# Dorothy-2016/rgbd360

Hardware: AMD Instinct MI355X
Metric: registered Frame360 pairs/sec @ 8×640×480; ICP-reduce HBM GB/s vs roofline (higher is better)
Workload: dtype f32

## Files before the change

### include/rgbd360_hip.h

```cpp
#ifndef RGBD360_HIP_H
#define RGBD360_HIP_H
#include <stddef.h>
#include <stdint.h>

#ifdef __cplusplus
extern "C" {
#endif

#define R360_NUM_SENSORS 8
#define R360_MAX_PYR 6

typedef struct r360_ctx r360_ctx;
typedef struct r360_calib r360_calib;
typedef struct r360_frame r360_frame;

int         r360_ctx_create(int device, r360_ctx** out);
void        r360_ctx_destroy(r360_ctx* ctx);
int         r360_ctx_sync(r360_ctx* ctx);
void*       r360_ctx_stream(r360_ctx* ctx);
const char* r360_last_error(void);
const char* r360_version(void);
const char* r360_data_dir(void);

int  r360_calib_create(r360_ctx* ctx, int rows, int cols, r360_calib** out);
// ... 253 lines not shown
    float pbmap_info[36];
    int   dense_rc;
    float pose[16];
    float hessian[36];
    r360_icp_stats stats;
} r360_pair_result;

int r360_batch_register(r360_batch* b, const r360_pair_job* jobs, int n, size_t max_match_planes, int mode,
                        int min_matches, float min_area, const r360_icp_params* p, r360_pair_result* out);

int r360_track_frame(r360_batch* b, r360_frame* const* kfs, int n_kf, r360_frame* frame, int num_check,
                     int no_assoc_threshold, size_t max_match_planes, int mode, int* chosen,
                     r360_pair_result* result, r360_pair_result* cand);

typedef struct {
    int   label, count, start_idx, n_contour, n_fit;
    float centroid[3], cov[9], model[4], curvature;
} r360_region;
int r360_frame_get_cloud(r360_frame* f, float* xyz4, uint8_t* rgb4, float* nrm4, float* dist);
int r360_frame_get_labels(r360_frame* f, int* lab, int* labf);
int r360_frame_get_regions(r360_frame* f, int sensor, r360_region* out, int cap, int* n);
int r360_frame_segment_eval(r360_frame* f, const float* xyz4, const float* nrm, int nrm_comps, const uint8_t* rgb4,
                            int* err_code);
int r360_frame_get_region_detail(r360_frame* f, int sensor, int region, int64_t* stats, float* bounds,
                                 float* contour4, int cap, int* n_contour);

typedef struct r360_comm r360_comm;
int  r360_comm_unique_id(uint8_t id[128]);
int  r360_comm_init(int device, int nranks, int rank, const uint8_t id[128], r360_comm** out);
void r360_comm_destroy(r360_comm* c);
int  r360_comm_allgather(r360_comm* c, const void* send, void* recv, size_t bytes);
int  r360_comm_allreduce_max(r360_comm* c, double* v, int n);

int  r360_dev_alloc(int device, size_t bytes, void** out);
int  r360_dev_free(void* p);
int  r360_dev_copy(void* dst, const void* src, size_t bytes, int kind);

int r360_synth_frame(const r360_calib* calib, uint32_t seed, const float rig_pose[16],
                     uint8_t* bgr8, uint16_t* depth8);
int r360_synth_frame_rt(int rows, int cols, const float* rt8, uint32_t seed, const float rig_pose[16],
                        uint8_t* bgr8, uint16_t* depth8);
int r360_synth_path_pose(uint32_t seed, int frame, float pose_out[16]);

int r360_proj_check(const float* X, const float* Y, const float* Z, int n, int nRows, int nCols,
                    unsigned long long* mismatches, unsigned long long* fallbacks);
int r360_proj_check_pose(const float* lx, const float* ly, const float* lz, int n, const float pose[16], int nRows,
// ... 201 lines not shown
```

### rgbd360_amd/__init__.py

```python
from __future__ import annotations

import ctypes as C
import os
import numpy as np

C = C

__all__ = [
    "lib", "Context", "Calib360", "Frame360", "RegisterPhotoICP", "RegisterRGBD360", "IcpParams", "IcpStats",
    "GicpParams", "GicpStats", "GeneralizedICP", "GraphParams", "GraphStats", "PoseGraph", "g2o_write", "g2o_read",
    "PHOTO_CONSISTENCY", "DEPTH_CONSISTENCY", "PHOTO_DEPTH", "synth_path_pose", "exp_se3",
    "LIB_PATH", "ABI_SYMBOLS", "Batch", "PairJob", "PairResult", "JOB_PBMAP_ONLY", "JOB_GATED", "JOB_ALWAYS",
    "TopoParams", "TopologicalMap", "Relocalizer", "topo_bisect", "topo_partition", "topo_partition_batch",
]

_HERE = os.path.dirname(os.path.abspath(__file__))
LIB_PATH = os.environ.get("R360_LIB") or os.path.join(_HERE, "lib", "librgbd360_hip.so")
REPO_ROOT = os.path.dirname(_HERE)

PHOTO_CONSISTENCY, DEPTH_CONSISTENCY, PHOTO_DEPTH = 0, 1, 2
BUILD_UNDISTORT, BUILD_SPHERE, BUILD_PYRAMID, BUILD_CLOUD, BUILD_PLANES = 1, 2, 4, 8, 16
BUILD_SENSOR_PYRAMID = 32
BUILD_LOCAL_PLANES = 64
BUILT_LEVEL0 = 256
# ... 303 lines not shown
    ("r360_match_params_load_ini", C.c_int, [C.c_char_p, C.POINTER(MatchParams)]),
    ("r360_ctx_set_match_params", C.c_int, [_P, C.POINTER(MatchParams)]),
    ("r360_ctx_get_match_params", C.c_int, [_P, C.POINTER(MatchParams)]),
    ("r360_ctx_match_stats", C.c_int, [_P, C.POINTER(C.c_long), C.POINTER(C.c_long), C.POINTER(C.c_long)]),
    ("r360_match_tree_search", C.c_int, [C.c_int, C.c_int, _P, _P, C.c_int, _P, C.c_long, _P, C.POINTER(C.c_long)]),
    ("r360_batch_set_match_params", C.c_int, [_P, C.POINTER(MatchParams)]),
    ("r360_register_pbmap", C.c_int, [_P, _P, _P, C.c_size_t, C.c_int, _FP, _FP, _IP, C.c_int, _IP, _FP, _FP, _FP]),
    ("r360_register", C.c_int, [_P, _P, _P, _FP, C.POINTER(IcpParams), C.c_size_t, C.c_int, _FP, _FP,
                                C.POINTER(IcpStats)]),
    ("r360_register_async", C.c_int, [_P, _P, _P, _FP, C.POINTER(IcpParams), C.c_size_t, C.c_int]),
    ("r360_register_result", C.c_int, [_P, _FP, _FP, C.POINTER(IcpStats)]),
    ("r360_pbmap_match_tables", C.c_int, [_P, _P, _P, C.c_size_t, C.c_int, _IP, _IP, _IP, _IP, _P, _P, C.c_int]),
    ("r360_batch_create", C.c_int, [C.c_int, C.c_int, C.POINTER(C.c_void_p)]),
    ("r360_batch_destroy", None, [_P]),
    ("r360_batch_lanes", C.c_int, [_P]),
    ("r360_batch_register", C.c_int, [_P, C.POINTER(PairJob), C.c_int, C.c_size_t, C.c_int, C.c_int, C.c_float,
                                      C.POINTER(IcpParams), C.POINTER(PairResult)]),
    ("r360_track_frame", C.c_int, [_P, C.POINTER(C.c_void_p), C.c_int, _P, C.c_int, C.c_int, C.c_size_t, C.c_int,
                                   _IP, C.POINTER(PairResult), C.POINTER(PairResult)]),
    ("r360_frame_get_cloud", C.c_int, [_P, _FP, _P, _FP, _FP]),
    ("r360_frame_get_labels", C.c_int, [_P, _IP, _IP]),
    ("r360_frame_get_regions", C.c_int, [_P, C.c_int, C.POINTER(Region), C.c_int, _IP]),
    ("r360_frame_segment_eval", C.c_int, [_P, _FP, _FP, C.c_int, _P, _IP]),
    ("r360_frame_get_region_detail", C.c_int, [_P, C.c_int, C.c_int, C.POINTER(C.c_int64), _FP, _FP, C.c_int, _IP]),
    ("r360_comm_unique_id", C.c_int, [_P]),
    ("r360_comm_init", C.c_int, [C.c_int, C.c_int, C.c_int, _P, C.POINTER(_P)]),
    ("r360_comm_destroy", None, [_P]),
    ("r360_comm_allgather", C.c_int, [_P, _P, _P, C.c_size_t]),
    ("r360_comm_allreduce_max", C.c_int, [_P, _DP, C.c_int]),
    ("r360_dev_alloc", C.c_int, [C.c_int, C.c_size_t, C.POINTER(_P)]),
    ("r360_dev_free", C.c_int, [_P]),
    ("r360_dev_copy", C.c_int, [_P, _P, C.c_size_t, C.c_int]),
    ("r360_synth_frame", C.c_int, [_P, C.c_uint32, _FP, _P, _P]),
    ("r360_synth_frame_rt", C.c_int, [C.c_int, C.c_int, _FP, C.c_uint32, _FP, _P, _P]),
    ("r360_synth_path_pose", C.c_int, [C.c_uint32, C.c_int, _FP]),
    ("r360_libm_eval", C.c_int, [_FP, _FP, _FP, C.c_int, _FP, _FP, C.c_int]),
    ("r360_rn_check", C.c_int, [C.c_uint, C.c_uint, C.POINTER(C.c_ulonglong)]),
    ("r360_rank6", C.c_int, [_FP, C.c_int, _IP]),
    ("r360_data_dir", C.c_char_p, []),
    ("r360_solve6", C.c_int, [_DP, _DP, C.c_int, _DP]),
    ("r360_proj_check_pose", C.c_int, [_FP, _FP, _FP, C.c_int, _FP, C.c_int, C.c_int, C.POINTER(C.c_ulonglong),
                                       C.POINTER(C.c_ulonglong)]),
    ("r360_proj_check", C.c_int, [_FP, _FP, _FP, C.c_int, C.c_int, C.c_int, C.POINTER(C.c_ulonglong),
                                  C.POINTER(C.c_ulonglong)]),
    ("r360_ctx_debug_stamps", C.c_int, [_P, C.POINTER(C.c_ulonglong)]),
    ("r360_ctx_kernel_time", C.c_int, [_P, C.c_int, C.POINTER(C.c_double), C.POINTER(C.c_long)]),
# ... 536 lines not shown
        n = C.c_int()
        arr = (Region * 64)()
        _check(lib().r360_frame_get_regions(self.h, sensor, arr, 64, C.byref(n)), "get_regions")
        return [dict(label=r.label, count=r.count, start_idx=r.start_idx, n_contour=r.n_contour, n_fit=r.n_fit,
                     centroid=np.array(r.centroid[:]), cov=np.array(r.cov[:]).reshape(3, 3),
                     model=np.array(r.model[:]), curvature=r.curvature) for r in arr[:n.value]]

    def segment_eval(self, xyz4: np.ndarray, nrm: np.ndarray, rgb4: np.ndarray) -> int:
        h, w = self.rows // 2, self.cols // 2
        xyz4 = np.ascontiguousarray(xyz4, np.float32)
        nrm = np.ascontiguousarray(nrm, np.float32)
        rgb4 = np.ascontiguousarray(rgb4, np.uint8)
        if xyz4.shape != (8, h, w, 4) or nrm.shape[:3] != (8, h, w) or nrm.shape[3] not in (3, 4) or \
                rgb4.shape != (8, h, w, 4):
            raise ValueError(f"segment_eval: fields of 8 x {h} x {w} expected")
        code = C.c_int(0)
        rc = lib().r360_frame_segment_eval(self.h, _fptr(xyz4), _fptr(nrm), nrm.shape[3], _vptr(rgb4), C.byref(code))
        if rc < 0:
            e = RuntimeError(f"segment_eval failed ({rc}): {lib().r360_last_error().decode()}")
            e.code = code.value
            raise e
        return rc

    def region_detail(self, sensor: int, region: int) -> dict:
        st = (C.c_int64 * 20)()
        bounds = np.zeros(6, np.float32)
        n = C.c_int()
        _check(lib().r360_frame_get_region_detail(self.h, sensor, region, st, _fptr(bounds), None, 0, C.byref(n)),
               "get_region_detail")
        contour = np.zeros((max(n.value, 1), 4), np.float32)
        if n.value:
            _check(lib().r360_frame_get_region_detail(self.h, sensor, region, None, None, _fptr(contour), n.value,
                                                      C.byref(n)), "get_region_detail")
        s2 = []
        for k in range(6):
            v = (int(st[4 + 2 * k]) & 0xFFFFFFFFFFFFFFFF) | ((int(st[5 + 2 * k]) & 0xFFFFFFFFFFFFFFFF) << 64)
            s2.append(v - (1 << 128) if v >> 127 else v)
        return dict(n=int(st[0]), s1=[int(st[1 + k]) for k in range(3)], s2=s2, c=[int(st[16 + k]) for k in range(4)],
                    bmin=bounds[:3].copy(), bmax=bounds[3:].copy(), contour=contour[:n.value].copy())

    def sphere(self):
        bgr = np.zeros((self.sph_rows, self.sph_cols, 3), np.uint8)
        dep = np.zeros((self.sph_rows, self.sph_cols), np.uint16)
        _check(lib().r360_frame_get_sphere(self.h, _vptr(bgr), _vptr(dep)), "get_sphere")
        return bgr, dep

# ... 131 lines not shown

    def match_tables(self, mode: int = PLANAR_3DoF, cap: int = 128):
        ns, nt = C.c_int(), C.c_int()
        sid, tid = np.zeros(cap, np.int32), np.zeros(cap, np.int32)
        un = np.zeros(cap * cap, np.uint8)
        words = (cap * cap + 63) // 64
        bi = np.zeros(cap * cap * words, np.uint64)
        _check(lib().r360_ctx_set_match_params(self.ctx.h, C.byref(self.match)), "set_match_params")
        w = _check(lib().r360_pbmap_match_tables(self.ctx.h, self.ref.h, self.trg.h, self.max_match_planes, mode,
                                                 C.byref(ns), C.byref(nt), sid.ctypes.data_as(_IP),
                                                 tid.ctypes.data_as(_IP), _vptr(un), _vptr(bi), cap), "match_tables")
        n, m = ns.value, nt.value
        return dict(sid=sid[:n].copy(), tid=tid[:m].copy(), unary=un[:n * m].reshape(n, m).copy(),
                    binary=bi[:n * m * w].reshape(n * m, w).copy(), words=w)


def frames_build(frames, flags: int = None):
    if flags is None:
        flags = BUILD_UNDISTORT | BUILD_CLOUD | BUILD_PLANES | BUILD_SPHERE | BUILD_PYRAMID
    arr = (C.c_void_p * len(frames))(*[f.h for f in frames])
    _check(lib().r360_frames_build(arr, len(frames), flags), "r360_frames_build")


def register(ctx: "Context", ref: "Frame360", trg: "Frame360", guess=None, params: "IcpParams | None" = None,
             max_match_planes: int = 25, mode: int = PLANAR_3DoF):
    g = _mat16(np.eye(4) if guess is None else guess)
    pose, info = np.zeros(16, np.float32), np.zeros(36, np.float32)
    st = IcpStats()
    p = params if params is not None else IcpParams.default()
    rc = _check(lib().r360_register(ctx.h, ref.h, trg.h, _fptr(g), C.byref(p), max_match_planes, mode, _fptr(pose),
                                    _fptr(info), C.byref(st)), "register")
    return _from16(pose), info.reshape(6, 6).T.copy(), st, rc == 0


class Batch:

    def __init__(self, device: int = 0, lanes: int = 8):
        h = C.c_void_p()
        _check(lib().r360_batch_create(device, lanes, C.byref(h)), "r360_batch_create")
        self.h = h
        self.lanes = lib().r360_batch_lanes(h)

    def register_pairs(self, jobs, max_match_planes: int = 25, mode: int = PLANAR_3DoF, min_matches: int = 0,
                       min_area: float = 0.0, params: "IcpParams | None" = None) -> list[dict]:
        jobs = list(jobs)
        arr = (PairJob * max(1, len(jobs)))()
# ... 901 lines not shown
```

### rgbd360_amd/csrc/host/pbmap.cpp

```cpp
#include <hip/hip_runtime.h>

#include <algorithm>
#include <chrono>
#include <condition_variable>
#include <deque>
#include <mutex>
#include <string>
#include <thread>
#include <cmath>
#include <cstdio>
#include <cstdlib>
#include <cstring>
#include <map>
#include <zlib.h>
#include <set>
#include <vector>

#include "../r360_internal.h"


int launch_match_tables(r360_ctx* ctx, hipStream_t stream, const float* d_desc, int ns, int nt, int mode,
                        uint8_t* d_unary, unsigned long long* d_bin, int words);

namespace {
// ... 1560 lines not shown
extern "C" int r360_frame_get_regions(r360_frame* f, int sensor, r360_region* out, int cap, int* n) {
    if (int rc = ready(f)) return rc;
    CHECK_ARG(f->pl.cloud, "frame planes were loaded, not built: no per-sensor regions");
    CHECK_ARG(sensor >= 0 && sensor < 8, "sensor out of range");
    PlaneBufs& P = f->pl;
    const int nm = P.h_nmodels[sensor];
    if (n) *n = nm;
    for (int m = 0; m < nm && m < cap && out; ++m) {
        const PlaneOut& O = P.h_out[sensor * R360_MAX_MODELS + m];
        r360_region& r = out[m];
        r.label = O.model.label;
        r.count = (int)O.stats.n;
        r.start_idx = O.start;
        r.n_contour = O.n_contour;
        r.n_fit = O.model.n_fit;
        for (int k = 0; k < 3; ++k) r.centroid[k] = O.model.centroid[k];
        for (int k = 0; k < 9; ++k) r.cov[k] = O.model.cov[k];
        for (int k = 0; k < 4; ++k) r.model[k] = O.model.v[k];
        r.curvature = O.model.curvature;
    }
    return 0;
}

extern "C" int r360_frame_segment_eval(r360_frame* f, const float* xyz4, const float* nrm, int nrm_comps,
                                       const uint8_t* rgb4, int* err_code) {
    CHECK_ARG(f && xyz4 && nrm && rgb4 && (nrm_comps == 3 || nrm_comps == 4), "segment_eval: bad arguments");
    if (bind_device(f->ctx->device)) return -1;
    CHECK_ARG(f->rows > 0, "a sphere-only frame has no sensor images");
    planes_join(f);
    if (plane_bufs_alloc(f)) return -1;
    r360_ctx* ctx = f->ctx;
    hipStream_t st = ctx->stream;
    PlaneBufs& P = f->pl;
    const int w = P.w, h = P.h, rows = f->rows, cols = f->cols;
    const size_t T = 8 * (size_t)w * h;
    std::vector<uint8_t> bgr((size_t)8 * rows * cols * 3, 0);
    for (int s = 0; s < 8; ++s)
        for (int r = 0; r < h; ++r)
            for (int c = 0; c < w; ++c) {
                const uint8_t* q = rgb4 + 4 * (((size_t)s * h + r) * w + c);
                uint8_t* d = bgr.data() + (((size_t)s * rows + 2 * r + 1) * cols + 2 * c + 1) * 3;
                d[0] = q[2]; d[1] = q[1]; d[2] = q[0];
            }
    std::vector<float> n4;
    if (nrm_comps == 3) {
        n4.resize(4 * T);
        for (size_t i = 0; i < T; ++i) {
            for (int k = 0; k < 3; ++k) n4[4 * i + k] = nrm[3 * i + k];
            n4[4 * i + 3] = 0.f;
        }
    }
    if (hipEvent_t e = f->bgr_wait()) R360_HIP(hipEventSynchronize(e));
    R360_HIP(hipStreamSynchronize(st));
    f->bgr_split = false;
    R360_HIP(hipMemcpy(f->d_bgr, bgr.data(), bgr.size(), hipMemcpyHostToDevice));
    R360_HIP(hipMemcpy(P.cloud, xyz4, sizeof(float4) * T, hipMemcpyHostToDevice));
    R360_HIP(hipMemcpy(P.nrm, nrm_comps == 3 ? n4.data() : nrm, sizeof(float4) * T, hipMemcpyHostToDevice));
    const PlaneGeom G = plane_geom(f);
    long cells, entries, groups;
    vox_scratch_need(G, &cells, &entries, &groups);
    if (ctx_vhash_reserve(ctx, cells, entries, groups)) return -1;
    PlaneBatch B;
    std::memset(&B, 0, sizeof B);
    B.f[0] = plane_dev(f, VoxScratch{ctx->d_vhash, (unsigned long long)ctx->vhash_cap, ctx->d_vlist, ctx->d_vcnt});
    P.ticket.reset();
    delete f->pbmap;
    f->pbmap = nullptr;
    delete f->local;
    f->local = nullptr;
    f->built = 0;
    if (launch_segment_inputs(B, 1, G, st)) return -1;
    if (launch_segmentation(B, 1, G, st, ctx, nullptr)) return -1;
    if (launch_plane_publish(B, 1, st)) return -1;
    R360_HIP(hipEventRecord(P.done, st));
    R360_HIP(hipStreamSynchronize(st));
    f->built = R360_BUILD_CLOUD | R360_BUILD_PLANES;
    if (err_code) *err_code = P.h_nmodels[8];
    if (planes_capacity_ok(f)) {
        P.worker_rc = -1;
        P.worker_err = r360_last_error();
        return -1;
    }
    P.worker_rc = 0;
    P.worker_err.clear();
    f->pbmap = new PbMapHost;
    return 0;
}

extern "C" int r360_frame_get_region_detail(r360_frame* f, int sensor, int region, int64_t* stats, float* bounds,
                                            float* contour4, int cap, int* n_contour) {
    if (int rc = ready(f)) return rc;
    CHECK_ARG(f->pl.cloud, "frame planes were loaded, not built: no per-sensor regions");
    CHECK_ARG(sensor >= 0 && sensor < 8, "sensor out of range");
    PlaneBufs& P = f->pl;
    CHECK_ARG(region >= 0 && region < P.h_nmodels[sensor], "region out of range");
    const PlaneOut& O = P.h_out[sensor * R360_MAX_MODELS + region];
    if (stats) {
        stats[0] = O.stats.n;
        for (int k = 0; k < 3; ++k) stats[1 + k] = O.stats.s1[k];
        for (int k = 0; k < 6; ++k) {
            const unsigned __int128 u = (unsigned __int128)O.stats.s2[k];
            stats[4 + 2 * k] = (int64_t)(unsigned long long)u;
            stats[5 + 2 * k] = (int64_t)(unsigned long long)(u >> 64);
        }
        for (int k = 0; k < 4; ++k) stats[16 + k] = O.stats.c[k];
    }
    if (bounds)
        for (int k = 0; k < 3; ++k) { bounds[k] = O.bmin[k]; bounds[3 + k] = O.bmax[k]; }
// ... 135 lines not shown
```

### rgbd360_amd/csrc/kernels/plane_seg.hip

```cpp
#include <cstdio>
#include <cstdlib>
#include <cstring>
#include <type_traits>
#include "../r360_internal.h"
#include "../plane_math.h"

namespace {

__device__ __forceinline__ bool isfin(float v) { return __builtin_isfinite(v); }

__device__ __forceinline__ int ld(const int* p) { return __hip_atomic_load(p, __ATOMIC_RELAXED, __HIP_MEMORY_SCOPE_AGENT); }

__device__ int find_root(int* parent, int x) {
    int p = ld(parent + x);
    while (p != x) {
        const int gp = ld(parent + p);
        if (gp != p) __hip_atomic_store(parent + x, gp, __ATOMIC_RELAXED, __HIP_MEMORY_SCOPE_AGENT);
        x = gp;
        p = ld(parent + x);
    }
    return x;
}

__device__ void unite(int* parent, int a, int b) {
// ... 906 lines not shown
    int8_t* B = bnd + (long)s * R360_REFINE_BANDS * w;
    int* Fl = flag + s * R360_REFINE_BANDS;
    for (int i = 1; i < nb; ++i) {
        const int b = DIR > 0 ? i : nb - 1 - i;
        const int prev = b - DIR;
        __builtin_amdgcn_fence(__ATOMIC_RELEASE, "workgroup");
        __builtin_amdgcn_wave_barrier();
        __builtin_amdgcn_fence(__ATOMIC_ACQUIRE, "workgroup");
        if (!__builtin_amdgcn_readfirstlane(Fl[prev])) continue;
        const int r0 = b * rb, r1 = min(h, r0 + rb);
        refine_band<K, DIR>(Sin + s * N, Sout + s * N, MK + s * N, w, h, r0, r1, B + (long)prev * w, B + (long)b * w,
                            Fl + b, true);
    }
}
template <int K, int DIR>
__global__ void __launch_bounds__(64) k_refine_p2(const PlaneBatch B, int w, int h, int rb, int nb) {
    const PlaneDev& D = B.f[blockIdx.z];
    d_refine_p2<K, DIR>(DIR > 0 ? D.state : D.state2, DIR > 0 ? D.state2 : D.state, D.mask, w, h, rb, nb, D.rbnd, D.rflag);
}


constexpr int RW_PF = 8;

__device__ __forceinline__ void d_refine_skew(const int8_t* __restrict__ S, const unsigned long long* __restrict__ MK, int w, int h,
                              uint16_t* __restrict__ code, unsigned long long* __restrict__ msk, int* __restrict__ fb) {
    const long N = (long)w * h, SK = (long)(h + w - 1) * h, total = 8 * SK;
    if (blockIdx.x == 0 && threadIdx.x < 24) fb[threadIdx.x] = 0;
    for (long d = blockIdx.x * (long)blockDim.x + threadIdx.x; d < total; d += (long)gridDim.x * blockDim.x) {
        const int s = (int)(d / SK);
        const long q = d - (long)s * SK;
        const int k = (int)(q / h), r = (int)(q - (long)k * h);
        const int c = k - r;
        if (c < 0 || c >= w) continue;
        const int j = r * w + c;
        const long i = (long)s * N + j;
        const int8_t* O = S + (long)s * N;
        const bool c1 = r >= 1 && c <= w - 2 && O[(r - 1) * w + c + 1] != -1;
        const bool c2 = r <= h - 2 && (c >= 1 ? O[(r + 1) * w + c - 1] != -1 : O[r * w + w - 1] != -1);
        code[d] = (uint16_t)((uint8_t)O[j] | (c1 ? 0x100 : 0) | (c2 ? 0x200 : 0));
        msk[d] = MK[i];
    }
}
__global__ void k_refine_skew(const PlaneBatch B, int w, int h) {
    const PlaneDev& D = B.f[blockIdx.z];
    d_refine_skew(D.state, D.mask, w, h, D.rcode, D.rmsk, D.rflag);
}


__device__ __forceinline__ bool mbit(unsigned long long m, int v) { return (v >= 0) & (((m >> (v & 63)) & 1ull) != 0); }

constexpr int RW_MAX_REDO = 64;

template <int DIR>
__device__ __forceinline__ void d_refine_wave(const uint16_t* __restrict__ code_all,
                                                      const unsigned long long* __restrict__ msk_all,
                                                      int8_t* __restrict__ f1_all, int8_t* __restrict__ f2_all,
                                                      int* __restrict__ fb, int w, int h) {
    __shared__ int xch[2][16];
    __shared__ int8_t wasm[1024], wdet[1024];
    __shared__ int s_red, s_min;
    __shared__ int chg[2][16];
    const int s = blockIdx.x;
    const int r = threadIdx.x, lane = r & 63, wv = r >> 6, nw = blockDim.x >> 6;
    const long SK = (long)(h + w - 1) * h;
    const uint16_t* code = code_all + s * SK;
    const unsigned long long* msk = msk_all + s * SK;
    int8_t* f1 = f1_all + s * SK;
    int8_t* f2 = f2_all + s * SK;
// ... 416 lines not shown
template <int DIR, int NW>
__global__ void __launch_bounds__(64 * NW) k_refine_pipe(const PlaneBatch B, int w, int h, int narrow_max) {
    const PlaneDev& D = B.f[blockIdx.z];
    d_refine_pipe<DIR, NW>(D.rcode, D.rmsk, D.rf1, D.rf2, D.nmodels, D.rflag, w, h, narrow_max);
}


__device__ __forceinline__ void d_refine_unskew(const int8_t* __restrict__ f2_all, int8_t* __restrict__ S_all,
                                const int* __restrict__ fb, int w, int h) {
    const long N = (long)w * h, SK = (long)(h + w - 1) * h, total = 8 * N;
    for (long i = blockIdx.x * (long)blockDim.x + threadIdx.x; i < total; i += (long)gridDim.x * blockDim.x) {
        const int s = (int)(i / N);
        if (fb[s]) continue;
        const int j = (int)(i - (long)s * N), r = j / w, c = j - r * w;
        S_all[i] = f2_all[s * SK + (long)(r + c) * h + r];
    }
}
__global__ void k_refine_unskew(const PlaneBatch B, int w, int h) {
    const PlaneDev& D = B.f[blockIdx.z];
    d_refine_unskew(D.rf2, D.state, D.rflag, w, h);
}


template <int K>
__device__ __forceinline__ void d_refine_fb(const int8_t* __restrict__ f1_all, const int8_t* __restrict__ f2_all,
                                                 int8_t* __restrict__ S_all,
                                                 const unsigned long long* __restrict__ MK, const int* __restrict__ fb,
                                                 int w, int h) {
    const int s = blockIdx.x;
    if (fb[16 + s]) {
        refine_sweeps<K>(S_all, MK, w, h, s, 3);
        return;
    }
    const int r0 = fb[s] - 1;
    if (r0 < 0) return;
    const long N = (long)w * h, SK = (long)(h + w - 1) * h;
    for (long j = threadIdx.x; j < N; j += 64) {
        const int r = (int)(j / w), c = (int)(j - (long)r * w);
        S_all[s * N + j] = (r <= r0 ? f1_all : f2_all)[s * SK + (long)(r + c) * h + r];
    }
    __builtin_amdgcn_fence(__ATOMIC_RELEASE, "workgroup");
    __builtin_amdgcn_wave_barrier();
    __builtin_amdgcn_fence(__ATOMIC_ACQUIRE, "workgroup");
    refine_sweeps<K>(S_all, MK, w, h, s, 2, r0 + 1);
}
template <int K>
__global__ void __launch_bounds__(64) k_refine_fb(const PlaneBatch B, int w, int h) {
    const PlaneDev& D = B.f[blockIdx.z];
    d_refine_fb<K>(D.rf1, D.rf2, D.state, D.mask, D.rflag, w, h);
}


__device__ __forceinline__ void d_refine_final(const int8_t* __restrict__ state, const int* __restrict__ lab, int N,
                               const PlaneModel* __restrict__ models, int* __restrict__ labf) {
    const long total = 8L * N;
    for (long i = blockIdx.x * (long)blockDim.x + threadIdx.x; i < total; i += (long)gridDim.x * blockDim.x) {
        const int s = (int)(i / N);
        const int st = state[i];
        labf[i] = st >= 0 ? models[s * R360_MAX_MODELS + st].label : (st == -2 ? lab[i] : -1);
    }
}
__global__ void k_refine_final(const PlaneBatch B, int N) {
    const PlaneDev& D = B.f[blockIdx.z];
    d_refine_final(D.state, D.lab, N, D.models, D.labf);
}


__device__ __forceinline__ void d_nbmask(const int* __restrict__ labf, int w, int h, uint8_t* __restrict__ nb,
                         const RegionPart* __restrict__ gpart, const int* __restrict__ nmodels,
                         PlaneOut* __restrict__ out) {
    const int N = w * h;
    const long total = 8L * N;
// ... 544 lines not shown
        if (keep) dst[off + (int)__builtin_amdgcn_mbcnt_hi((unsigned)(bal >> 32), __builtin_amdgcn_mbcnt_lo((unsigned)bal, 0u))] = v;
        __syncthreads();
        if (tid == 0) for (int w = 0; w < VOXH_TPB / 64; ++w) s_base += s_wc[w];
        __syncthreads();
    }
    return s_base;
}

__global__ void __launch_bounds__(VOXH_TPB) k_hullpre(const PlaneBatch B) {
    const PlaneDev& D = B.f[blockIdx.z];
    const int q = blockIdx.x, s = q / R360_MAX_MODELS, m = q % R360_MAX_MODELS;
    if (m >= D.nmodels[s]) return;
    PlaneOut& O = D.out[q];
    int kept = 0;
    if (O.n_contour > 0)
        kept = d_hullpre(D.contour_dev + O.contour_off, D.contour + O.contour_off, O.n_contour, O.model);
    else if (O.n_vox > 0 && D.totals[3] != 0)
        kept = d_hullpre(D.vox_dev + O.vox_off, D.vox + O.vox_off, O.n_vox, O.model);
    if (threadIdx.x == 0) O.hull_n = kept;
}
}


int refine_band_rows(int h) {
    static const int env = R360_KNOB("R360_REFINE_ROWS", -99);
    int rb = env >= -2 ? env : -1;
    if (rb < 0) return h <= 1024 ? rb : 0;
    if (rb > 0 && (h + rb - 1) / rb > R360_REFINE_BANDS) rb = (h + R360_REFINE_BANDS - 1) / R360_REFINE_BANDS;
    return rb;
}

int launch_refine_sweeps(const PlaneBatch& B, int F, hipStream_t st, int w, int h, int rb, bool wave_bufs) {
    const int K = (w + 63) / 64;
    const unsigned nf = (unsigned)F;
    if (rb < 0 && (w < 2 || h > 1024 || !wave_bufs)) rb = 0;
    if (rb < 0) {
        const long slots = 8L * (h + w - 1) * h;
        hipLaunchKernelGGL(k_refine_skew, dim3((unsigned)((slots + 255) / 256), 1, nf), dim3(256), 0, st, B, w, h);
        const int tpb = 64 * ((h + 63) / 64);
        const int narrow_max = 30;
        if (rb == -1 && h <= 64 * RP_MAXB && w <= RP_MAXW) {
            if (h <= 256) {
                hipLaunchKernelGGL((k_refine_pipe<1, 4>), dim3(8, 1, nf), dim3(tpb), 0, st, B, w, h, narrow_max);
                hipLaunchKernelGGL((k_refine_pipe<-1, 4>), dim3(8, 1, nf), dim3(tpb), 0, st, B, w, h, narrow_max);
            } else {
                hipLaunchKernelGGL((k_refine_pipe<1, RP_MAXB>), dim3(8, 1, nf), dim3(tpb), 0, st, B, w, h, narrow_max);
                hipLaunchKernelGGL((k_refine_pipe<-1, RP_MAXB>), dim3(8, 1, nf), dim3(tpb), 0, st, B, w, h, narrow_max);
            }
        } else {
            hipLaunchKernelGGL(k_refine_wave<1>, dim3(8, 1, nf), dim3(tpb), 0, st, B, w, h);
            hipLaunchKernelGGL(k_refine_wave<-1>, dim3(8, 1, nf), dim3(tpb), 0, st, B, w, h);
        }
        hipLaunchKernelGGL(k_refine_unskew, dim3((unsigned)((8L * w * h + 255) / 256), 1, nf), dim3(256), 0, st, B, w, h);
        switch (K) {
#define R360_FB_CASE(k) case k: hipLaunchKernelGGL(k_refine_fb<k>, dim3(8, 1, nf), dim3(64), 0, st, B, w, h); break;
            R360_FB_CASE(1) R360_FB_CASE(2) R360_FB_CASE(3) R360_FB_CASE(4) R360_FB_CASE(5)
            R360_FB_CASE(6) R360_FB_CASE(7) R360_FB_CASE(8) R360_FB_CASE(9) R360_FB_CASE(10)
#undef R360_FB_CASE
            default: r360_set_error("refine: cloud width %d > 640 unsupported", w); return -1;
        }
        R360_HIP(hipGetLastError());
        return 0;
    }
    if (rb > 0 && (h + rb - 1) / rb > R360_REFINE_BANDS) { r360_set_error("refine: %d rows per band too few", rb); return -2; }
    const int nb = rb > 0 ? (h + rb - 1) / rb : 0;
    switch (K) {
#define R360_REFINE_CASE(k)                                                                                     \
    case k:                                                                                                     \
        if (rb == 0) { hipLaunchKernelGGL(k_refine<k>, dim3(8, 1, nf), dim3(64), 0, st, B, w, h); break; }      \
        hipLaunchKernelGGL((k_refine_p1<k, 1>), dim3(nb, 8, nf), dim3(64), 0, st, B, w, h, rb);                 \
        hipLaunchKernelGGL((k_refine_p2<k, 1>), dim3(8, 1, nf), dim3(64), 0, st, B, w, h, rb, nb);              \
        hipLaunchKernelGGL((k_refine_p1<k, -1>), dim3(nb, 8, nf), dim3(64), 0, st, B, w, h, rb);                \
        hipLaunchKernelGGL((k_refine_p2<k, -1>), dim3(8, 1, nf), dim3(64), 0, st, B, w, h, rb, nb);             \
        break;
        R360_REFINE_CASE(1) R360_REFINE_CASE(2) R360_REFINE_CASE(3) R360_REFINE_CASE(4) R360_REFINE_CASE(5)
        R360_REFINE_CASE(6) R360_REFINE_CASE(7) R360_REFINE_CASE(8) R360_REFINE_CASE(9) R360_REFINE_CASE(10)
#undef R360_REFINE_CASE
        default: r360_set_error("refine: cloud width %d > 640 unsupported", w); return -1;
    }
    R360_HIP(hipGetLastError());
    return 0;
}

template <bool MODEL>
int launch_gm(int px, long total, const PlaneBatch& B, int F, hipStream_t st, int N) {
    const unsigned blocks = (unsigned)((total + px - 1) / px);
    const int exp = 0;
    switch (px) {
#define R360_GM_CASE(cpw)                                                                                         \
    case 256 * cpw:                                                                                               \
        hipLaunchKernelGGL((k_gm<MODEL, cpw>), dim3(blocks, 1, (unsigned)F), dim3(GM_TPB), 0, st, B, N, exp);    \
        return 0;
        R360_GM_CASE(1) R360_GM_CASE(2) R360_GM_CASE(4) R360_GM_CASE(8) R360_GM_CASE(16)
#undef R360_GM_CASE
    }
    r360_set_error("segmentation: R360_GM_PX=%d (256, 512, 1024, 2048 or 4096)", px);
    return -1;
}

int launch_segmentation_geom(const PlaneBatch& B, int F, const PlaneGeom& G, hipStream_t st, r360_ctx* tctx) {
    const int w = G.w, h = G.h, N = w * h;
    const long total = 8L * N;
// ... 3 lines not shown
    int slot = timing_begin(tctx, "k_ccl");
    hipLaunchKernelGGL(k_ccl_local, dim3((h + CCL_ROWS - 1) / CCL_ROWS, 8, nf), dim3(CCL_TPB), sizeof(int) * CCL_ROWS * w,
                       st, B, w, h, ang_thr);
    {
        const long edges = 8L * ((h - 1) / CCL_ROWS) * w;
        if (edges > 0)
            hipLaunchKernelGGL(k_ccl_border, dim3((unsigned)((edges + 255) / 256), 1, nf), dim3(256), 0, st, B, w, h, ang_thr);
    }
    const int nch = (N + NUMC - 1) / NUMC;
    hipLaunchKernelGGL(k_ccl_flatten, dim3(nch, 8, nf), dim3(NUMC), 0, st, B, N);
    hipLaunchKernelGGL(k_ccl_number, dim3(nch, 8, nf), dim3(NUMC), 0, st, B, N);
    hipLaunchKernelGGL(k_ccl_label, dim3(blocks, 1, nf), dim3(256), 0, st, B, N);
    timing_end(tctx, slot);
    R360_HIP(hipGetLastError());
    slot = timing_begin(tctx, "k_plane_fit");
    hipLaunchKernelGGL(k_big_count, dim3(nch, 8, nf), dim3(NUMC), 0, st, B, N, 80);
    hipLaunchKernelGGL(k_big_list, dim3(nch, 8, nf), dim3(NUMC), 0, st, B, N, 80, R360_MAX_BIG);
    static const int gm_px = R360_KNOB("R360_GM_PX", GM_PX);
    if (launch_gm<false>(gm_px, total, B, F, st, N)) return -1;
    hipLaunchKernelGGL(k_plane_fit, dim3(8, 1, nf), dim3(PF_TPB), 0, st, B, R360_MAX_BIG, 0.001f, N);
    timing_end(tctx, slot);
    R360_HIP(hipGetLastError());
    slot = timing_begin(tctx, "k_refine");
    hipLaunchKernelGGL(k_refine_init, dim3(blocks, 1, nf), dim3(256), 0, st, B, N);
    if (launch_refine_sweeps(B, F, st, w, h, refine_band_rows(h), true)) return -1;
    hipLaunchKernelGGL(k_refine_final, dim3(blocks, 1, nf), dim3(256), 0, st, B, N);
    timing_end(tctx, slot);
    R360_HIP(hipGetLastError());
    return 0;
}

int launch_segmentation_model(const PlaneBatch& B, int F, const PlaneGeom& G, hipStream_t st, r360_ctx* tctx) {
    const int w = G.w, h = G.h, N = w * h;
    const long total = 8L * N;
    const int blocks = (int)((total + 255) / 256);
    const unsigned nf = (unsigned)F;
    static const int gm_px = R360_KNOB("R360_GM_PX", GM_PX);
    int slot = timing_begin(tctx, "k_model_stats");
    if (launch_rgb(B, F, G, st)) return -1;
    if (launch_gm<true>(gm_px, total, B, F, st, N)) return -1;
    hipLaunchKernelGGL(k_nbmask, dim3(std::max(blocks, 20 * 8 * R360_MAX_MODELS / 256), 1, nf), dim3(256), 0, st, B, w, h);
    if (N <= TR_NB_MAX) hipLaunchKernelGGL(k_trace<true>, dim3(8, 1, nf), dim3(TR_TPB), 0, st, B, w, h);
    else hipLaunchKernelGGL(k_trace<false>, dim3(8, 1, nf), dim3(TR_TPB), 0, st, B, w, h);
    long cells, entries, groups;
    vox_scratch_need(G, &cells, &entries, &groups);
    const int vox_px = (int)(entries / groups);
    hipLaunchKernelGGL(k_alloc, dim3(1, 1, nf), dim3(512), 0, st, B);
    timing_end(tctx, slot);
    R360_HIP(hipGetLastError());
// ... 96 lines not shown
    R360_HIP(hipMemcpy(MK, mask, sizeof(unsigned long long) * T, hipMemcpyHostToDevice));
    uint16_t* code; unsigned long long* msk; int8_t *f1, *f2;
    const size_t SK = 8 * (size_t)(h + w - 1) * h;
    R360_HIP(hipMalloc(&code, sizeof(uint16_t) * SK));
    R360_HIP(hipMalloc(&msk, sizeof(unsigned long long) * SK));
    R360_HIP(hipMalloc(&f1, SK));
    R360_HIP(hipMalloc(&f2, SK));
    int nmh[8], *nm;
    for (int s = 0; s < 8; ++s) {
        int top = 0;
        for (size_t i = (size_t)s * w * h; i < (size_t)(s + 1) * w * h; ++i) {
            if (state[i] + 1 > top) top = state[i] + 1;
            if (mask[i]) top = std::max(top, 64 - __builtin_clzll(mask[i]));
        }
        nmh[s] = top;
    }
    R360_HIP(hipMalloc(&nm, sizeof(nmh)));
    R360_HIP(hipMemcpy(nm, nmh, sizeof(nmh), hipMemcpyHostToDevice));
    PlaneBatch B;
    std::memset(&B, 0, sizeof B);
    PlaneDev& D = B.f[0];
    D.state = S; D.state2 = S2; D.mask = MK; D.rbnd = bnd; D.rflag = flag;
    D.rcode = code; D.rmsk = msk; D.rf1 = f1; D.rf2 = f2; D.nmodels = nm;
    int rc = launch_refine_sweeps(B, 1, 0, w, h, rb, true);
    if (rc == 0) {
        R360_HIP(hipMemcpy(out, S, T, hipMemcpyDeviceToHost));
        if (rb < 0 && w >= 2 && h <= 1024) {
            int fbh[16];
            R360_HIP(hipMemcpy(fbh, flag, sizeof(fbh), hipMemcpyDeviceToHost));
            for (int k = 0; k < 8; ++k) rc += (fbh[k] != 0 || fbh[8 + k] != 0);
            if (R360_KNOB_STR("R360_REFINE_TRACE"))
                for (int k = 0; k < 8; ++k) fprintf(stderr, "refine sensor %d: re-runs %d fallback row %d\n", k, fbh[8 + k], fbh[k] - 1);
        }
    }
    (void)hipFree(S); (void)hipFree(S2); (void)hipFree(MK); (void)hipFree(bnd); (void)hipFree(flag); (void)hipFree(nm);
    (void)hipFree(code); (void)hipFree(msk); (void)hipFree(f1); (void)hipFree(f2);
    return rc;
}
```

Before: 2006.

## Fuse refine init into skew prep and label finalize into unskew kernel

In the wave refine path, the frame pipeline now folds refine state initialisation (model assignment and point-to-plane masks) into a per-pixel prep kernel that writes the skewed code and mask buffers directly. The separate unskew and final-label kernels are replaced by a finish kernel that writes both state and final labels, with the fallback kernel also emitting labels. This removes full-image passes and kernel launches over state, mask and label buffers. It also adds a batched segment_eval API, a refine-state readback and a forced-fallback test hook, which increases scope and adds risk of label mismatches on the fallback paths.

Result: faster. 2035, median of 6 (+1.4%).

```diff
diff --git a/include/rgbd360_hip.h b/include/rgbd360_hip.h
--- a/include/rgbd360_hip.h
+++ b/include/rgbd360_hip.h
@@ -299,6 +299,10 @@
 int r360_frame_get_regions(r360_frame* f, int sensor, r360_region* out, int cap, int* n);
 int r360_frame_segment_eval(r360_frame* f, const float* xyz4, const float* nrm, int nrm_comps, const uint8_t* rgb4,
                             int* err_code);
+int r360_frames_segment_eval(r360_frame* const* frames, int n, const float* xyz4, const float* nrm, int nrm_comps,
+                             const uint8_t* rgb4, int* err_codes);
+int r360_frame_get_refine_states(r360_frame* f, int8_t* state, int* flags);
+void r360_refine_force_fallback(uint64_t sensor_mask, int first_sweep);
 int r360_frame_get_region_detail(r360_frame* f, int sensor, int region, int64_t* stats, float* bounds,
                                  float* contour4, int cap, int* n_contour);
 
diff --git a/rgbd360_amd/__init__.py b/rgbd360_amd/__init__.py
--- a/rgbd360_amd/__init__.py
+++ b/rgbd360_amd/__init__.py
@@ -349,6 +349,9 @@
     ("r360_frame_get_labels", C.c_int, [_P, _IP, _IP]),
     ("r360_frame_get_regions", C.c_int, [_P, C.c_int, C.POINTER(Region), C.c_int, _IP]),
     ("r360_frame_segment_eval", C.c_int, [_P, _FP, _FP, C.c_int, _P, _IP]),
+    ("r360_frames_segment_eval", C.c_int, [C.POINTER(C.c_void_p), C.c_int, _FP, _FP, C.c_int, _P, _IP]),
+    ("r360_frame_get_refine_states", C.c_int, [_P, _P, _IP]),
+    ("r360_refine_force_fallback", None, [C.c_uint64, C.c_int]),
     ("r360_frame_get_region_detail", C.c_int, [_P, C.c_int, C.c_int, C.POINTER(C.c_int64), _FP, _FP, C.c_int, _IP]),
     ("r360_comm_unique_id", C.c_int, [_P]),
     ("r360_comm_init", C.c_int, [C.c_int, C.c_int, C.c_int, _P, C.POINTER(_P)]),
@@ -931,6 +934,13 @@
             raise e
         return rc
 
+    def refine_states(self):
+        state = np.zeros((8, self.rows // 2, self.cols // 2), np.int8)
+        flags = np.zeros(24, np.int32)
+        _check(lib().r360_frame_get_refine_states(self.h, state.ctypes.data, flags.ctypes.data_as(_IP)),
+               "get_refine_states")
+        return state, flags
+
     def region_detail(self, sensor: int, region: int) -> dict:
         st = (C.c_int64 * 20)()
         bounds = np.zeros(6, np.float32)
@@ -1108,6 +1118,30 @@
     _check(lib().r360_frames_build(arr, len(frames), flags), "r360_frames_build")
 
 
+def refine_force_fallback(sensor_mask: int = 0, first_sweep: bool = False):
+    lib().r360_refine_force_fallback(sensor_mask, int(first_sweep))
+
+
+def frames_segment_eval(frames, xyz4: np.ndarray, nrm: np.ndarray, rgb4: np.ndarray):
+    n = len(frames)
+    h, w = frames[0].rows // 2, frames[0].cols // 2
+    xyz4 = np.ascontiguousarray(xyz4, np.float32)
+    nrm = np.ascontiguousarray(nrm, np.float32)
+    rgb4 = np.ascontiguousarray(rgb4, np.uint8)
+    if xyz4.shape != (n, 8, h, w, 4) or nrm.shape[:4] != (n, 8, h, w) or nrm.shape[4] not in (3, 4) or \
+            rgb4.shape != (n, 8, h, w, 4):
+        raise ValueError(f"frames_segment_eval: fields of {n} x 8 x {h} x {w} expected")
+    arr = (C.c_void_p * n)(*[f.h for f in frames])
+    codes = np.zeros(n, np.int32)
+    rc = lib().r360_frames_segment_eval(arr, n, _fptr(xyz4), _fptr(nrm), nrm.shape[4], _vptr(rgb4),
+                                        codes.ctypes.data_as(_IP))
+    if rc < 0:
+        e = RuntimeError(f"frames_segment_eval failed ({rc}): {lib().r360_last_error().decode()}")
+        e.codes = codes
+        raise e
+    return codes
+
+
 def register(ctx: "Context", ref: "Frame360", trg: "Frame360", guess=None, params: "IcpParams | None" = None,
              max_match_planes: int = 25, mode: int = PLANAR_3DoF):
     g = _mat16(np.eye(4) if guess is None else guess)
diff --git a/rgbd360_amd/csrc/host/pbmap.cpp b/rgbd360_amd/csrc/host/pbmap.cpp
--- a/rgbd360_amd/csrc/host/pbmap.cpp
+++ b/rgbd360_amd/csrc/host/pbmap.cpp
@@ -1606,68 +1606,109 @@
     return 0;
 }
 
+extern "C" int r360_frames_segment_eval(r360_frame* const* frames, int n, const float* xyz4, const float* nrm,
+                                        int nrm_comps, const uint8_t* rgb4, int* err_codes) {
+    CHECK_ARG(frames && n >= 1 && n <= R360_PLANE_BATCH && xyz4 && nrm && rgb4 && (nrm_comps == 3 || nrm_comps == 4),
+              "segment_eval: bad arguments");
+    for (int i = 0; i < n; ++i) {
+        CHECK_ARG(frames[i] && frames[i]->rows > 0, "a sphere-only frame has no sensor images");
+        CHECK_ARG(frames[i]->ctx == frames[0]->ctx && frames[i]->rows == frames[0]->rows && frames[i]->cols == frames[0]->cols,
+                  "segment_eval: frames of one context and size expected");
+        for (int j = 0; j < i; ++j) CHECK_ARG(frames[j] != frames[i], "segment_eval: a frame is listed twice");
+    }
+    r360_ctx* ctx = frames[0]->ctx;
+    if (bind_device(ctx->device)) return -1;
+    hipStream_t st = ctx->stream;
+    if ((int)ctx->bvox.size() < R360_PLANE_BATCH - 1) ctx->bvox.resize(R360_PLANE_BATCH - 1);
+    PlaneBatch B;
+    std::memset(&B, 0, sizeof B);
+    PlaneGeom G{};
+    for (int i = 0; i < n; ++i) {
+        r360_frame* f = frames[i];
+        planes_join(f);
+        if (plane_bufs_alloc(f)) return -1;
+        PlaneBufs& P = f->pl;
+        const int w = P.w, h = P.h, rows = f->rows, cols = f->cols;
+        const size_t T = 8 * (size_t)w * h;
+        const float* fx = xyz4 + 4 * T * i;
+        const float* fn = nrm + (size_t)nrm_comps * T * i;
+        const uint8_t* fc = rgb4 + 4 * T * i;
+        std::vector<uint8_t> bgr((size_t)8 * rows * cols * 3, 0);
+        for (int s = 0; s < 8; ++s)
+            for (int r = 0; r < h; ++r)
+                for (int c = 0; c < w; ++c) {
+                    const uint8_t* q = fc + 4 * (((size_t)s * h + r) * w + c);
+                    uint8_t* d = bgr.data() + (((size_t)s * rows + 2 * r + 1) * cols + 2 * c + 1) * 3;
+                    d[0] = q[2]; d[1] = q[1]; d[2] = q[0];
+                }
+        std::vector<float> n4;
+        if (nrm_comps == 3) {
+            n4.resize(4 * T);
+            for (size_t k = 0; k < T; ++k) {
+                for (int q = 0; q < 3; ++q) n4[4 * k + q] = fn[3 * k + q];
+                n4[4 * k + 3] = 0.f;
+            }
+        }
+        if (hipEvent_t e = f->bgr_wait()) R360_HIP(hipEventSynchronize(e));
+        R360_HIP(hipStreamSynchronize(st));
+        f->bgr_split = false;
+        R360_HIP(hipMemcpy(f->d_bgr, bgr.data(), bgr.size(), hipMemcpyHostToDevice));
+        R360_HIP(hipMemcpy(P.cloud, fx, sizeof(float4) * T, hipMemcpyHostToDevice));
+        R360_HIP(hipMemcpy(P.nrm, nrm_comps == 3 ? n4.data() : fn, sizeof(float4) * T, hipMemcpyHostToDevice));
+        G = plane_geom(f);
+        long cells, entries, groups;
+        vox_scratch_need(G, &cells, &entries, &groups);
+        if (ctx_vhash_reserve(ctx, cells, entries, groups)) return -1;
+        VoxScratch vs{ctx->d_vhash, (unsigned long long)ctx->vhash_cap, ctx->d_vlist, ctx->d_vcnt};
+        if (i > 0) {
+            if (vox_slot_reserve(ctx->bvox[i - 1], G, st)) return -1;
+            vs = ctx->bvox[i - 1].v;
+        }
+        B.f[i] = plane_dev(f, vs);
+        P.ticket.reset();
+        delete f->pbmap;
+        f->pbmap = nullptr;
+        delete f->local;
+        f->local = nullptr;
+        f->built = 0;
+    }
+    if (launch_segment_inputs(B, n, G, st)) return -1;
+    if (launch_segmentation(B, n, G, st, ctx, nullptr)) return -1;
+    if (launch_plane_publish(B, n, st)) return -1;
+    for (int i = 0; i < n; ++i) R360_HIP(hipEventRecord(frames[i]->pl.done, st));
+    R360_HIP(hipStreamSynchronize(st));
+    int rc = 0;
+    for (int i = 0; i < n; ++i) {
+        r360_frame* f = frames[i];
+        PlaneBufs& P = f->pl;
+        f->built = R360_BUILD_CLOUD | R360_BUILD_PLANES;
+        if (err_codes) err_codes[i] = P.h_nmodels[8];
+        if (planes_capacity_ok(f)) {
+            P.worker_rc = -1;
+            P.worker_err = r360_last_error();
+            rc = -1;
+            continue;
+        }
+        P.worker_rc = 0;
+        P.worker_err.clear();
+        f->pbmap = new PbMapHost;
+    }
+    return rc;
+}
+
 extern "C" int r360_frame_segment_eval(r360_frame* f, const float* xyz4, const float* nrm, int nrm_comps,
                                        const uint8_t* rgb4, int* err_code) {
-    CHECK_ARG(f && xyz4 && nrm && rgb4 && (nrm_comps == 3 || nrm_comps == 4), "segment_eval: bad arguments");
-    if (bind_device(f->ctx->device)) return -1;
-    CHECK_ARG(f->rows > 0, "a sphere-only frame has no sensor images");
-    planes_join(f);
-    if (plane_bufs_alloc(f)) return -1;
-    r360_ctx* ctx = f->ctx;
-    hipStream_t st = ctx->stream;
+    CHECK_ARG(f, "segment_eval: bad arguments");
+    return r360_frames_segment_eval(&f, 1, xyz4, nrm, nrm_comps, rgb4, err_code);
+}
+
+extern "C" int r360_frame_get_refine_states(r360_frame* f, int8_t* state, int* flags) {
+    CHECK_ARG(state && flags, "get_refine_states: null output");
+    if (int rc = ready(f)) return rc;
+    CHECK_ARG(f->pl.cloud, "frame planes were loaded, not built: no refinement states");
     PlaneBufs& P = f->pl;
-    const int w = P.w, h = P.h, rows = f->rows, cols = f->cols;
-    const size_t T = 8 * (size_t)w * h;
-    std::vector<uint8_t> bgr((size_t)8 * rows * cols * 3, 0);
-    for (int s = 0; s < 8; ++s)
-        for (int r = 0; r < h; ++r)
-            for (int c = 0; c < w; ++c) {
-                const uint8_t* q = rgb4 + 4 * (((size_t)s * h + r) * w + c);
-                uint8_t* d = bgr.data() + (((size_t)s * rows + 2 * r + 1) * cols + 2 * c + 1) * 3;
-                d[0] = q[2]; d[1] = q[1]; d[2] = q[0];
-            }
-    std::vector<float> n4;
-    if (nrm_comps == 3) {
-        n4.resize(4 * T);
-        for (size_t i = 0; i < T; ++i) {
-            for (int k = 0; k < 3; ++k) n4[4 * i + k] = nrm[3 * i + k];
-            n4[4 * i + 3] = 0.f;
-        }
-    }
-    if (hipEvent_t e = f->bgr_wait()) R360_HIP(hipEventSynchronize(e));
-    R360_HIP(hipStreamSynchronize(st));
-    f->bgr_split = false;
-    R360_HIP(hipMemcpy(f->d_bgr, bgr.data(), bgr.size(), hipMemcpyHostToDevice));
-    R360_HIP(hipMemcpy(P.cloud, xyz4, sizeof(float4) * T, hipMemcpyHostToDevice));
-    R360_HIP(hipMemcpy(P.nrm, nrm_comps == 3 ? n4.data() : nrm, sizeof(float4) * T, hipMemcpyHostToDevice));
-    const PlaneGeom G = plane_geom(f);
-    long cells, entries, groups;
-    vox_scratch_need(G, &cells, &entries, &groups);
-    if (ctx_vhash_reserve(ctx, cells, entries, groups)) return -1;
-    PlaneBatch B;
-    std::memset(&B, 0, sizeof B);
-    B.f[0] = plane_dev(f, VoxScratch{ctx->d_vhash, (unsigned long long)ctx->vhash_cap, ctx->d_vlist, ctx->d_vcnt});
-    P.ticket.reset();
-    delete f->pbmap;
-    f->pbmap = nullptr;
-    delete f->local;
-    f->local = nullptr;
-    f->built = 0;
-    if (launch_segment_inputs(B, 1, G, st)) return -1;
-    if (launch_segmentation(B, 1, G, st, ctx, nullptr)) return -1;
-    if (launch_plane_publish(B, 1, st)) return -1;
-    R360_HIP(hipEventRecord(P.done, st));
-    R360_HIP(hipStreamSynchronize(st));
-    f->built = R360_BUILD_CLOUD | R360_BUILD_PLANES;
-    if (err_code) *err_code = P.h_nmodels[8];
-    if (planes_capacity_ok(f)) {
-        P.worker_rc = -1;
-        P.worker_err = r360_last_error();
-        return -1;
-    }
-    P.worker_rc = 0;
-    P.worker_err.clear();
-    f->pbmap = new PbMapHost;
+    R360_HIP(hipMemcpy(state, P.state, 8 * (size_t)P.w * P.h, hipMemcpyDeviceToHost));
+    R360_HIP(hipMemcpy(flags, P.rflag, sizeof(int) * 24, hipMemcpyDeviceToHost));
     return 0;
 }
 
diff --git a/rgbd360_amd/csrc/kernels/plane_seg.hip b/rgbd360_amd/csrc/kernels/plane_seg.hip
--- a/rgbd360_amd/csrc/kernels/plane_seg.hip
+++ b/rgbd360_amd/csrc/kernels/plane_seg.hip
@@ -952,28 +952,53 @@
 
 constexpr int RW_PF = 8;
 
-__device__ __forceinline__ void d_refine_skew(const int8_t* __restrict__ S, const unsigned long long* __restrict__ MK, int w, int h,
-                              uint16_t* __restrict__ code, unsigned long long* __restrict__ msk, int* __restrict__ fb) {
-    const long N = (long)w * h, SK = (long)(h + w - 1) * h, total = 8 * SK;
-    if (blockIdx.x == 0 && threadIdx.x < 24) fb[threadIdx.x] = 0;
-    for (long d = blockIdx.x * (long)blockDim.x + threadIdx.x; d < total; d += (long)gridDim.x * blockDim.x) {
-        const int s = (int)(d / SK);
-        const long q = d - (long)s * SK;
-        const int k = (int)(q / h), r = (int)(q - (long)k * h);
-        const int c = k - r;
-        if (c < 0 || c >= w) continue;
-        const int j = r * w + c;
-        const long i = (long)s * N + j;
+template <bool INIT>
+__device__ __forceinline__ void d_refine_prep(const float4* __restrict__ cloud, const int* __restrict__ lab,
+                                              const PlaneModel* __restrict__ models, const int* __restrict__ nmodels,
+                                              int8_t* __restrict__ S, unsigned long long* __restrict__ MK, int w, int h,
+                                              uint16_t* __restrict__ code, unsigned long long* __restrict__ msk,
+                                              int* __restrict__ fb) {
+    const int s = blockIdx.y, N = w * h;
+    if (blockIdx.x == 0 && s == 0 && threadIdx.x < 24) fb[threadIdx.x] = 0;
+    const int j = blockIdx.x * blockDim.x + threadIdx.x;
+    if (j >= N) return;
+    const int r = j / w, c = j - r * w;
+    const long i = (long)s * N + j;
+    const long d = (long)s * (h + w - 1) * h + (long)(r + c) * h + r;
+    const int up = (r - 1) * w + c + 1, dn = c >= 1 ? (r + 1) * w + c - 1 : r * w + w - 1;
+    int st;
+    unsigned long long bits = 0;
+    bool c1 = r >= 1 && c <= w - 2, c2 = r <= h - 2;
+    if (INIT) {
+        const int* L8 = lab + (long)s * N;
+        const int L = L8[j];
+        const int nm = nmodels[s];
+        const PlaneModel* M = models + s * R360_MAX_MODELS;
+        st = L < 0 ? -1 : -2;
+        const float4 p = cloud[i];
+        for (int m = 0; m < nm; ++m) {
+            if (L >= 0 && M[m].label == L) st = m;
+            const double ptp = fabs((double)(M[m].v[0] * p.x + M[m].v[1] * p.y + M[m].v[2] * p.z + M[m].v[3]));
+            if (ptp < (double)0.02f) bits |= 1ull << m;
+        }
+        S[i] = (int8_t)st;
+        MK[i] = bits;
+        c1 = c1 && L8[up] >= 0;
+        c2 = c2 && L8[dn] >= 0;
+    } else {
         const int8_t* O = S + (long)s * N;
-        const bool c1 = r >= 1 && c <= w - 2 && O[(r - 1) * w + c + 1] != -1;
-        const bool c2 = r <= h - 2 && (c >= 1 ? O[(r + 1) * w + c - 1] != -1 : O[r * w + w - 1] != -1);
-        code[d] = (uint16_t)((uint8_t)O[j] | (c1 ? 0x100 : 0) | (c2 ? 0x200 : 0));
-        msk[d] = MK[i];
-    }
-}
-__global__ void k_refine_skew(const PlaneBatch B, int w, int h) {
-    const PlaneDev& D = B.f[blockIdx.z];
-    d_refine_skew(D.state, D.mask, w, h, D.rcode, D.rmsk, D.rflag);
+        st = O[j];
+        bits = MK[i];
+        c1 = c1 && O[up] != -1;
+        c2 = c2 && O[dn] != -1;
+    }
+    code[d] = (uint16_t)((uint8_t)(int8_t)st | (c1 ? 0x100 : 0) | (c2 ? 0x200 : 0));
+    msk[d] = bits;
+}
+template <bool INIT>
+__global__ void __launch_bounds__(256) k_refine_prep(const PlaneBatch B, int w, int h) {
+    const PlaneDev& D = B.f[blockIdx.z];
+    d_refine_prep<INIT>(D.cloud, D.lab, D.models, D.nmodels, D.state, D.mask, w, h, D.rcode, D.rmsk, D.rflag);
 }
 
 
@@ -1436,32 +1461,62 @@
 }
 
 
-template <int K>
+__device__ __forceinline__ void d_refine_finish(const int8_t* __restrict__ f2_all, int8_t* __restrict__ S_all,
+                                                const int* __restrict__ fb, const int* __restrict__ lab,
+                                                const PlaneModel* __restrict__ models, int* __restrict__ labf, int w,
+                                                int h) {
+    const int s = blockIdx.y, N = w * h;
+    if (fb[s] != 0 || fb[16 + s] != 0) return;
+    const int j = blockIdx.x * blockDim.x + threadIdx.x;
+    if (j >= N) return;
+    const int r = j / w, c = j - r * w;
+    const long i = (long)s * N + j;
+    const int st = f2_all[(long)s * (h + w - 1) * h + (long)(r + c) * h + r];
+    S_all[i] = (int8_t)st;
+    labf[i] = st >= 0 ? models[s * R360_MAX_MODELS + st].label : (st == -2 ? lab[i] : -1);
+}
+__global__ void __launch_bounds__(256) k_refine_finish(const PlaneBatch B, int w, int h) {
+    const PlaneDev& D = B.f[blockIdx.z];
+    d_refine_finish(D.rf2, D.state, D.rflag, D.lab, D.models, D.labf, w, h);
+}
+
+
+template <int K, bool LABF>
 __device__ __forceinline__ void d_refine_fb(const int8_t* __restrict__ f1_all, const int8_t* __restrict__ f2_all,
                                                  int8_t* __restrict__ S_all,
                                                  const unsigned long long* __restrict__ MK, const int* __restrict__ fb,
-                                                 int w, int h) {
+                                                 const int* __restrict__ lab, const PlaneModel* __restrict__ models,
+                                                 int* __restrict__ labf, int w, int h) {
     const int s = blockIdx.x;
+    const long N = (long)w * h, SK = (long)(h + w - 1) * h;
     if (fb[16 + s]) {
         refine_sweeps<K>(S_all, MK, w, h, s, 3);
-        return;
-    }
-    const int r0 = fb[s] - 1;
-    if (r0 < 0) return;
-    const long N = (long)w * h, SK = (long)(h + w - 1) * h;
-    for (long j = threadIdx.x; j < N; j += 64) {
-        const int r = (int)(j / w), c = (int)(j - (long)r * w);
-        S_all[s * N + j] = (r <= r0 ? f1_all : f2_all)[s * SK + (long)(r + c) * h + r];
-    }
-    __builtin_amdgcn_fence(__ATOMIC_RELEASE, "workgroup");
-    __builtin_amdgcn_wave_barrier();
-    __builtin_amdgcn_fence(__ATOMIC_ACQUIRE, "workgroup");
-    refine_sweeps<K>(S_all, MK, w, h, s, 2, r0 + 1);
-}
-template <int K>
+    } else {
+        const int r0 = fb[s] - 1;
+        if (r0 < 0) return;
+        for (long j = threadIdx.x; j < N; j += 64) {
+            const int r = (int)(j / w), c = (int)(j - (long)r * w);
+            S_all[s * N + j] = (r <= r0 ? f1_all : f2_all)[s * SK + (long)(r + c) * h + r];
+        }
+        __builtin_amdgcn_fence(__ATOMIC_RELEASE, "workgroup");
+        __builtin_amdgcn_wave_barrier();
+        __builtin_amdgcn_fence(__ATOMIC_ACQUIRE, "workgroup");
+        refine_sweeps<K>(S_all, MK, w, h, s, 2, r0 + 1);
+    }
+    if (LABF) {
+        __builtin_amdgcn_fence(__ATOMIC_RELEASE, "workgroup");
+        __builtin_amdgcn_wave_barrier();
+        __builtin_amdgcn_fence(__ATOMIC_ACQUIRE, "workgroup");
+        for (long j = threadIdx.x; j < N; j += 64) {
+            const int st = S_all[s * N + j];
+            labf[s * N + j] = st >= 0 ? models[s * R360_MAX_MODELS + st].label : (st == -2 ? lab[s * N + j] : -1);
+        }
+    }
+}
+template <int K, bool LABF>
 __global__ void __launch_bounds__(64) k_refine_fb(const PlaneBatch B, int w, int h) {
     const PlaneDev& D = B.f[blockIdx.z];
-    d_refine_fb<K>(D.rf1, D.rf2, D.state, D.mask, D.rflag, w, h);
+    d_refine_fb<K, LABF>(D.rf1, D.rf2, D.state, D.mask, D.rflag, D.lab, D.models, D.labf, w, h);
 }
 
 
@@ -2052,6 +2107,30 @@
 }
 
 
+static unsigned long long g_force_fb_mask = 0;
+static int g_force_fb_first = 0;
+
+namespace {
+__global__ void k_refine_force_fb(const PlaneBatch B, int w, int h, unsigned long long mask, int first_sweep) {
+    const int f = blockIdx.x, s = blockIdx.y;
+    if (!((mask >> (8 * f + s)) & 1ull)) return;
+    const PlaneDev& D = B.f[f];
+    int* fb = D.rflag;
+    if (!first_sweep) {
+        if (threadIdx.x == 0) fb[s] = (h - 1) / 2 + 1;
+        return;
+    }
+    if (threadIdx.x == 0) { fb[s] = h - 1; fb[16 + s] = 1; }
+    const long SK = (long)(h + w - 1) * h;
+    for (long q = threadIdx.x; q < SK; q += blockDim.x) { D.rf1[s * SK + q] = -1; D.rf2[s * SK + q] = -1; }
+}
+}
+
+extern "C" void r360_refine_force_fallback(uint64_t sensor_mask, int first_sweep) {
+    g_force_fb_mask = sensor_mask;
+    g_force_fb_first = first_sweep;
+}
+
 int refine_band_rows(int h) {
     static const int env = R360_KNOB("R360_REFINE_ROWS", -99);
     int rb = env >= -2 ? env : -1;
@@ -2060,13 +2139,16 @@
     return rb;
 }
 
-int launch_refine_sweeps(const PlaneBatch& B, int F, hipStream_t st, int w, int h, int rb, bool wave_bufs) {
+int launch_refine_sweeps(const PlaneBatch& B, int F, hipStream_t st, int w, int h, int rb, bool wave_bufs, bool frame) {
     const int K = (w + 63) / 64;
     const unsigned nf = (unsigned)F;
+    const int N = w * h;
+    const dim3 px_grid((unsigned)((N + 255) / 256), 8, nf);
+    const int blocks = (int)((8L * N + 255) / 256);
     if (rb < 0 && (w < 2 || h > 1024 || !wave_bufs)) rb = 0;
     if (rb < 0) {
-        const long slots = 8L * (h + w - 1) * h;
-        hipLaunchKernelGGL(k_refine_skew, dim3((unsigned)((slots + 255) / 256), 1, nf), dim3(256), 0, st, B, w, h);
+        if (frame) hipLaunchKernelGGL(k_refine_prep<true>, px_grid, dim3(256), 0, st, B, w, h);
+        else hipLaunchKernelGGL(k_refine_prep<false>, px_grid, dim3(256), 0, st, B, w, h);
         const int tpb = 64 * ((h + 63) / 64);
         const int narrow_max = 30;
         if (rb == -1 && h <= 64 * RP_MAXB && w <= RP_MAXW) {
@@ -2081,9 +2163,16 @@
             hipLaunchKernelGGL(k_refine_wave<1>, dim3(8, 1, nf), dim3(tpb), 0, st, B, w, h);
             hipLaunchKernelGGL(k_refine_wave<-1>, dim3(8, 1, nf), dim3(tpb), 0, st, B, w, h);
         }
-        hipLaunchKernelGGL(k_refine_unskew, dim3((unsigned)((8L * w * h + 255) / 256), 1, nf), dim3(256), 0, st, B, w, h);
+        if (frame && g_force_fb_mask && h >= 2)
+            hipLaunchKernelGGL(k_refine_force_fb, dim3(nf, 8), dim3(256), 0, st, B, w, h, g_force_fb_mask, g_force_fb_first);
+        if (frame) hipLaunchKernelGGL(k_refine_finish, px_grid, dim3(256), 0, st, B, w, h);
+        else hipLaunchKernelGGL(k_refine_unskew, dim3((unsigned)blocks, 1, nf), dim3(256), 0, st, B, w, h);
         switch (K) {
-#define R360_FB_CASE(k) case k: hipLaunchKernelGGL(k_refine_fb<k>, dim3(8, 1, nf), dim3(64), 0, st, B, w, h); break;
+#define R360_FB_CASE(k)                                                                                         \
+    case k:                                                                                                     \
+        if (frame) hipLaunchKernelGGL((k_refine_fb<k, true>), dim3(8, 1, nf), dim3(64), 0, st, B, w, h);        \
+        else hipLaunchKernelGGL((k_refine_fb<k, false>), dim3(8, 1, nf), dim3(64), 0, st, B, w, h);             \
+        break;
             R360_FB_CASE(1) R360_FB_CASE(2) R360_FB_CASE(3) R360_FB_CASE(4) R360_FB_CASE(5)
             R360_FB_CASE(6) R360_FB_CASE(7) R360_FB_CASE(8) R360_FB_CASE(9) R360_FB_CASE(10)
 #undef R360_FB_CASE
@@ -2094,6 +2183,7 @@
     }
     if (rb > 0 && (h + rb - 1) / rb > R360_REFINE_BANDS) { r360_set_error("refine: %d rows per band too few", rb); return -2; }
     const int nb = rb > 0 ? (h + rb - 1) / rb : 0;
+    if (frame) hipLaunchKernelGGL(k_refine_init, dim3(blocks, 1, nf), dim3(256), 0, st, B, N);
     switch (K) {
 #define R360_REFINE_CASE(k)                                                                                     \
     case k:                                                                                                     \
@@ -2108,6 +2198,7 @@
 #undef R360_REFINE_CASE
         default: r360_set_error("refine: cloud width %d > 640 unsupported", w); return -1;
     }
+    if (frame) hipLaunchKernelGGL(k_refine_final, dim3(blocks, 1, nf), dim3(256), 0, st, B, N);
     R360_HIP(hipGetLastError());
     return 0;
 }
@@ -2157,9 +2248,7 @@
     timing_end(tctx, slot);
     R360_HIP(hipGetLastError());
     slot = timing_begin(tctx, "k_refine");
-    hipLaunchKernelGGL(k_refine_init, dim3(blocks, 1, nf), dim3(256), 0, st, B, N);
-    if (launch_refine_sweeps(B, F, st, w, h, refine_band_rows(h), true)) return -1;
-    hipLaunchKernelGGL(k_refine_final, dim3(blocks, 1, nf), dim3(256), 0, st, B, N);
+    if (launch_refine_sweeps(B, F, st, w, h, refine_band_rows(h), true, true)) return -1;
     timing_end(tctx, slot);
     R360_HIP(hipGetLastError());
     return 0;
@@ -2302,7 +2391,7 @@
     PlaneDev& D = B.f[0];
     D.state = S; D.state2 = S2; D.mask = MK; D.rbnd = bnd; D.rflag = flag;
     D.rcode = code; D.rmsk = msk; D.rf1 = f1; D.rf2 = f2; D.nmodels = nm;
-    int rc = launch_refine_sweeps(B, 1, 0, w, h, rb, true);
+    int rc = launch_refine_sweeps(B, 1, 0, w, h, rb, true, false);
     if (rc == 0) {
         R360_HIP(hipMemcpy(out, S, T, hipMemcpyDeviceToHost));
         if (rb < 0 && w >= 2 && h <= 1024) {
```
